# hasindu2008/cornetto

Measured on AMD Instinct MI355X. Metric: Gbases/s scanned (telowin+sdust+boringbits), higher is better.
Workload: dtype u8/u16 integer

## Files before the change

cornetto_amd/csrc/cov.hip:

```cpp
#include <algorithm>
#include <cmath>

#include "common.hpp"
#include "scan.hpp"
#include "tiles.hpp"
#include "ivlmerge.hpp"
#include "internal.hpp"

namespace {

constexpr int CB_THREADS = 256;
#ifndef CN_CB_PARTS
#define CN_CB_PARTS 2
#endif
constexpr int CB_PARTS = CN_CB_PARTS;
constexpr int CB_MAX_INC_LDS = 128;

struct CbArgs {
    const uint16_t *depth, *mq;
    const int64_t *ctg_off;
    const int32_t *ctg_len;
    const int2 *tiles;
    int32_t inc, r;
    uint2 *pre;
    uint2 *head;
    int64_t n_tiles;
    const int4 *tmeta;
    uint2 *tile_tot32;
    ulonglong2 *tile_tot64;
};

typedef unsigned short cb_us2 __attribute__((ext_vector_type(2)));
__device__ __forceinline__ uint32_t add_u16x2(uint32_t acc, uint32_t pair)
{
    const cb_us2 ones = {1, 1};
    return __builtin_amdgcn_udot2(__builtin_bit_cast(cb_us2, pair), ones, acc, false);
}

typedef unsigned int cb_u4 __attribute__((ext_vector_type(4)));

template <bool STAGE, int INC, int NT = 1>
__global__ __launch_bounds__(CB_THREADS) void cov_blocks(CbArgs A)
{
    __builtin_amdgcn_s_setprio(CN_STREAM_PRIO);

    extern __shared__ __attribute__((aligned(16))) uint8_t smem[];
    __shared__ uint32_t wsum[2][CB_THREADS / 64];
    __shared__ unsigned long long wsum64[2][CB_THREADS / 64];

    const int t = threadIdx.x;
    const int inc = INC ? INC : A.inc, r = A.r;
    constexpr int PBc = CB_THREADS / CB_PARTS;
    constexpr int NVIc = INC ? (PBc * INC / 8 + CB_THREADS - 1) / CB_THREADS : 4;
    cb_u4 pre_all[NT][2][CB_PARTS][NVIc];
    if (STAGE && INC) {
#pragma unroll
        for (int ti = 0; ti < NT; ++ti) {
            const int64_t tix = (int64_t)blockIdx.x * NT + ti;
            if (tix >= A.n_tiles) continue;
            int2 tl;
            int ln;
            int64_t of;
            if (A.tmeta) {
                const int4 m0 = A.tmeta[2 * tix], m1 = A.tmeta[2 * tix + 1];
                tl = make_int2(m0.x, m0.y); ln = m0.z; of = (int64_t)(((unsigned long long)(uint32_t)m1.y << 32) | (uint32_t)m1.x);
            } else {
                tl = A.tiles[tix]; ln = A.ctg_len[tl.x]; of = A.ctg_off[tl.x];
            }
            const int64_t e0l = (int64_t)tl.y * inc;
            const int nvec = PBc * inc / 8;
#pragma unroll
            for (int which = 0; which < 2; ++which)
#pragma unroll
                for (int part = 0; part < CB_PARTS; ++part) {
                    const int64_t pe0 = e0l + (int64_t)part * PBc * inc;
                    const int64_t left = ((int64_t)ln - pe0) * 2;
                    const uint32_t nrec = left <= 0 ? 0u : (uint32_t)(left < (int64_t)nvec * 16 ? (left + 15) & ~15LL : (int64_t)nvec * 16);
                    const __amdgpu_buffer_rsrc_t rs = __builtin_amdgcn_make_buffer_rsrc((void *)((which ? A.mq : A.depth) + of + pe0), 0, (int)nrec, 0x00020000);
#pragma unroll
                    for (int k = 0; k < NVIc; ++k) pre_all[ti][which][part][k] = __builtin_amdgcn_raw_buffer_load_b128(rs, (t + k * CB_THREADS) * 16, 0, 0);
                }
        }
    }
#pragma unroll
  for (int ti = 0; ti < NT; ++ti) {
    const int64_t tix = (int64_t)blockIdx.x * NT + ti;
    if (tix >= A.n_tiles) break;
    if (ti) __syncthreads();
    int2 tile;
    int len;
    int64_t off;
    if (A.tmeta) {
        const int4 m0 = A.tmeta[2 * tix], m1 = A.tmeta[2 * tix + 1];
        tile = make_int2(m0.x, m0.y); len = m0.z; off = (int64_t)(((unsigned long long)(uint32_t)m1.y << 32) | (uint32_t)m1.x);
    } else {
        tile = A.tiles[tix]; len = A.ctg_len[tile.x]; off = A.ctg_off[tile.x];
    }
    const int64_t e0 = (int64_t)tile.y * inc;
    const int64_t p0 = e0 + (int64_t)t * inc;

    uint32_t fd = 0, fq = 0, hd = 0, hq = 0;
    unsigned long long xd = 0, xq = 0;
    if (STAGE) {
        uint16_t *sv = reinterpret_cast<uint16_t *>(smem);
        constexpr int PB = CB_THREADS / CB_PARTS;
        const int nvec = PB * inc / 8;
        const int base = (t % PB) * inc;
        const int nval = p0 >= len ? 0 : (int)(len - p0 < inc ? len - p0 : inc);
        const int nh = r < nval ? r : nval;
        constexpr int NVI = NVIc;
        auto &pre = pre_all[ti];
#pragma unroll
        for (int which = 0; which < 2; ++which) {
#pragma unroll
            for (int part = 0; part < CB_PARTS; ++part) {
                const int64_t pe0 = e0 + (int64_t)part * PB * inc;
                const int64_t left = ((int64_t)len - pe0) * 2;
                const uint32_t nrec = left <= 0 ? 0u : (uint32_t)(left < (int64_t)nvec * 16 ? (left + 15) & ~15LL : (int64_t)nvec * 16);
                const __amdgpu_buffer_rsrc_t rs = __builtin_amdgcn_make_buffer_rsrc((void *)((which ? A.mq : A.depth) + off + pe0), 0, (int)nrec, 0x00020000);
                if (which | part) __syncthreads();
                constexpr int NV = 4;
                if (INC) {
#pragma unroll
                    for (int k = 0; k < NVI; ++k) {
                        const int v = t + k * CB_THREADS;
                        if (v < nvec) reinterpret_cast<cb_u4 *>(sv)[v] = pre[which][part][k];
                    }
                } else
                for (int v0 = t; v0 < nvec; v0 += NV * CB_THREADS) {
                    cb_u4 a[NV];
#pragma unroll
                    for (int k = 0; k < NV; ++k) a[k] = __builtin_amdgcn_raw_buffer_load_b128(rs, (v0 + k * CB_THREADS) * 16, 0, 0);
#pragma unroll
                    for (int k = 0; k < NV; ++k) {
                        const int v = v0 + k * CB_THREADS;
                        if (v < nvec) reinterpret_cast<cb_u4 *>(sv)[v] = a[k];
                    }
                }
                __syncthreads();
                if (t / PB == part) {
                    uint32_t f = 0, hh = 0;
                    if (INC && (INC & 1) == 0 && nval == inc) {
                        const uint32_t *wd = reinterpret_cast<const uint32_t *>(sv + base);
#pragma unroll
                        for (int i = 0; i < (INC ? INC : 2) / 2; ++i) f = add_u16x2(f, wd[i]);
                    } else if (nval == inc && (inc & 1) == 0) {
                        const uint32_t *wd = reinterpret_cast<const uint32_t *>(sv + base);
                        for (int i = 0; i < inc / 2; ++i) f = add_u16x2(f, wd[i]);
                    } else {
#pragma clang loop vectorize(disable) unroll(disable)
                        for (int i = 0; i < nval; ++i) f += sv[base + i];
                    }
#pragma clang loop vectorize(disable) unroll(disable)
                    for (int i = 0; i < nh; ++i) hh += sv[base + i];
                    if (which) { fq = f; hq = hh; } else { fd = f; hd = hh; }
                }
            }
        }
        xd = fd;
        xq = fq;
    } else {
        const uint16_t *d = A.depth + off, *q = A.mq + off;
        for (int64_t p = p0; p < p0 + inc && p < len; ++p) {
            const uint32_t a = d[p], b = q[p];
            xd += a;
            xq += b;
            if (p - p0 < r) {
                hd += a;
                hq += b;
            }
        }
        fd = (uint32_t)xd;
        fq = (uint32_t)xq;
    }

    const int lane = t & 63, wv = t >> 6;
    uint32_t sdv, sqv;
    unsigned long long td = 0, tq = 0;
    if (STAGE) {
        sdv = cnwave::wave_incl_dpp(fd);
        sqv = cnwave::wave_incl_dpp(fq);
    } else {
        sdv = cnwave::wave_incl(fd, lane);
        sqv = cnwave::wave_incl(fq, lane);
        td = xd;
        tq = xq;
#pragma unroll
        for (int d = 32; d >= 1; d >>= 1) {
            td += ((unsigned long long)__shfl_xor((unsigned)(td >> 32), d) << 32) | __shfl_xor((unsigned)td, d);
            tq += ((unsigned long long)__shfl_xor((unsigned)(tq >> 32), d) << 32) | __shfl_xor((unsigned)tq, d);
        }
    }
    if (lane == 63) {
        wsum[0][wv] = sdv;
        wsum[1][wv] = sqv;
    }
    if (!STAGE && lane == 0) {
        wsum64[0][wv] = td;
        wsum64[1][wv] = tq;
    }
    __syncthreads();
    uint32_t pd = 0, pq = 0;
#pragma unroll
    for (int i = 0; i < CB_THREADS / 64; ++i)
        if (i < wv) {
            pd += wsum[0][i];
            pq += wsum[1][i];
        }
    A.pre[(size_t)tix * CB_THREADS + t] = make_uint2(sdv + pd, sqv + pq);
    if (A.r) A.head[(size_t)tix * CB_THREADS + t] = make_uint2(hd, hq);
    if (t == CB_THREADS - 1) {
        A.tile_tot32[tix] = make_uint2(sdv + pd, sqv + pq);
        ulonglong2 x;
        if (STAGE) {
            x.x = sdv + pd;
            x.y = sqv + pq;
        } else {
            x.x = wsum64[0][0] + wsum64[0][1] + wsum64[0][2] + wsum64[0][3];
            x.y = wsum64[1][0] + wsum64[1][1] + wsum64[1][2] + wsum64[1][3];
        }
        A.tile_tot64[tix] = x;
    }
  }
}

__global__ __launch_bounds__(256) void cov_total64(const ulonglong2 *tot64, int64_t n, unsigned long long *grand )
{
    __shared__ unsigned long long sa[4], sb[4];
    unsigned long long a = 0, b = 0;
    for (int64_t i = (int64_t)blockIdx.x * 256 + threadIdx.x; i < n; i += (int64_t)gridDim.x * 256) {
        const ulonglong2 v = tot64[i];
        a += v.x;
        b += v.y;
    }
#pragma unroll
    for (int d = 32; d >= 1; d >>= 1) {
        a += ((unsigned long long)__shfl_xor((unsigned)(a >> 32), d) << 32) | __shfl_xor((unsigned)a, d);
        b += ((unsigned long long)__shfl_xor((unsigned)(b >> 32), d) << 32) | __shfl_xor((unsigned)b, d);
    }
    if ((threadIdx.x & 63) == 0) {
        sa[threadIdx.x >> 6] = a;
        sb[threadIdx.x >> 6] = b;
    }
    __syncthreads();
    if (threadIdx.x == 0) {
        atomicAdd(&grand[0], sa[0] + sa[1] + sa[2] + sa[3]);
        atomicAdd(&grand[1], sb[0] + sb[1] + sb[2] + sb[3]);
    }
}

struct CwArgs {
    const uint2 *pre, *head;
    const uint32_t *toff_d, *toff_q;
    const int64_t *blk_off;
    const int32_t *ctg_len;
    const int32_t *n_reg;
    const int2 *tiles;
    int32_t w, inc, q, r;
    uint32_t w_magic, w_shift;
    int32_t mode;
    int32_t lo, hi, edge, min_len;
    double low_mq;
    cornetto_reg_t *regs;
    cornetto_regrec_t *sel;
    cornetto_regpk_t *pk;
    uint2 *tile_res;
};

__device__ __forceinline__ uint2 cw_prefix(const CwArgs &A, int64_t x)
{
    const uint2 b = A.pre[x];
    return make_uint2(b.x + A.toff_d[x >> 8], b.y + A.toff_q[x >> 8]);
}

__global__ __launch_bounds__(256) void cov_windows(CwArgs A)
{
    __builtin_amdgcn_s_setprio(CN_STREAM_PRIO);

    __shared__ uint32_t wcnt[4];
    const int t = threadIdx.x;
    const int2 tile = A.tiles[blockIdx.x];
    const int ctg = tile.x;
    const int len = A.ctg_len[ctg];
    const int j = tile.y + t;
    bool valid = j < A.n_reg[ctg];
    int st = 0, end = 0, depth = 0, mq = 0;
    bool sel = false;
    if (valid) {
        st = j * A.inc;
        end = st + A.w;
        if (end > len) end = len;
        const int64_t a = A.blk_off[ctg] + j;
        uint32_t sd = 0, sq = 0;
        if (A.q > 0) {
            const uint2 hi = cw_prefix(A, a + A.q - 1);
            uint2 lo = make_uint2(0, 0);
            if (a > 0) lo = cw_prefix(A, a - 1);
            sd = hi.x - lo.x;
            sq = hi.y - lo.y;
        }
        if (A.r) {
            const uint2 hb = A.head[a + A.q];
            sd += hb.x;
            sq += hb.y;
        }
        if (end - st == A.w && A.w_magic && (int32_t)(sd | sq) >= 0) {
            depth = (int32_t)(__umulhi(sd, A.w_magic) >> A.w_shift);
            mq = (int32_t)(__umulhi(sq, A.w_magic) >> A.w_shift);
        } else {
            depth = (int32_t)sd / (end - st);
            mq = (int32_t)sq / (end - st);
        }
        if (A.mode == 0) {
            A.regs[j] = cornetto_reg_t{st, end, depth, mq};
        } else {
            bool fun = depth < A.lo || depth > A.hi;
            if (!fun && !(A.low_mq <= 1.0 && depth > 0 && mq >= depth)) fun = ((double)mq / (double)depth) < A.low_mq;
            if (A.mode == 1) sel = len >= A.min_len && fun;
            else sel = len > A.min_len && st > A.edge && end < len - A.edge && !fun;
        }
    }
    if (A.mode == 0) return;
    const unsigned long long bal = __ballot(sel);
    const int lane = t & 63, wv = t >> 6;
    if (lane == 0) wcnt[wv] = (uint32_t)__popcll(bal);
    __syncthreads();
    uint32_t pre = 0, tot = 0;
#pragma unroll
    for (int i = 0; i < 4; ++i) {
        if (i < wv) pre += wcnt[i];
        tot += wcnt[i];
    }
    if (t == 0) A.tile_res[blockIdx.x] = make_uint2(blockIdx.x * 256u, tot);
    if (sel) {
        const size_t idx = (size_t)blockIdx.x * 256u + pre + __popcll(bal & ((1ull << lane) - 1ull));
        if (A.pk) A.pk[idx] = cornetto_regpk_t{st, (uint16_t)depth, (uint16_t)mq};
        else A.sel[idx] = cornetto_regrec_t{ctg, st, end, depth, mq};
    }
}

__global__ void cov_ctg_first(const uint32_t *ooff, const int32_t *first_tile, int32_t n_ctg, uint32_t n_tiles, const unsigned long long *total, uint32_t *out)
{
    const int32_t i = (int32_t)(blockIdx.x * blockDim.x + threadIdx.x);
    if (i >= n_ctg) return;
    const uint32_t t = (uint32_t)first_tile[i];
    out[i] = t < n_tiles ? ooff[t] : (uint32_t)*total;
}

template <int INTS>
__global__ __launch_bounds__(256) void cov_order(const int32_t *raw, const uint2 *tres, const uint32_t *ooff, int64_t n_tiles, int32_t *dst, const unsigned long long *total,
                                                 uint32_t cap)
{
    const int64_t t = (int64_t)blockIdx.x * 4 + (threadIdx.x >> 6);
    if (t >= n_tiles) return;
    if (*total > cap) return;
    const uint2 r = tres[t];
    const int32_t *src = raw + (size_t)r.x * INTS;
    int32_t *d = dst + (size_t)ooff[t] * INTS;
    const uint32_t nint = r.y * (uint32_t)INTS;
    for (uint32_t i = threadIdx.x & 63; i < nint; i += 64) d[i] = src[i];
}

__global__ __launch_bounds__(256) void cov_order_expand(const cornetto_regpk_t *raw, const uint2 *tres, const uint32_t *ooff, int64_t n_tiles, cornetto_regrec_t *dst,
                                                        const unsigned long long *total, uint32_t cap, const int2 *tiles, const int32_t *ctg_len, int32_t w)
{
    const int64_t t = (int64_t)blockIdx.x * 4 + (threadIdx.x >> 6);
    if (t >= n_tiles) return;
    if (*total > cap) return;
    const uint2 r = tres[t];
    const int32_t ctg = tiles[t].x, len = ctg_len[ctg];
    const cornetto_regpk_t *src = raw + r.x;
    cornetto_regrec_t *d = dst + ooff[t];
    for (uint32_t i = threadIdx.x & 63; i < r.y; i += 64) {
        const cornetto_regpk_t p = src[i];
        const int64_t e = (int64_t)p.st + w;
        d[i] = cornetto_regrec_t{ctg, p.st, e > len ? len : (int32_t)e, (int32_t)p.depth, (int32_t)p.mq_depth};
    }
}

int32_t n_reg_host(int32_t length, int32_t w, int32_t inc)
{
    int32_t n = (length - w + inc - 1) / inc + 1;
    return n < 1 ? 1 : n;
}

int32_t regs_assert_host(int32_t length, int32_t w, int32_t inc)
{
    const int64_t st = (int64_t)(n_reg_host(length, w, inc) - 1) * inc;
    int64_t end = st + w;
    if (end > length) end = length;
    if (!(st < end)) return 353;
    return end == length ? 0 : 368;
}

}

extern "C" {

int32_t cornetto_n_reg(int32_t length, int32_t window_size, int32_t window_inc)
{
    if (window_inc <= 0) return 0;
    return n_reg_host(length, window_size, window_inc);
}

int32_t cornetto_regs_assert(int32_t length, int32_t window_size, int32_t window_inc)
{
    if (window_inc <= 0) return 353;
    return regs_assert_host(length, window_size, window_inc);
}

int32_t cornetto_cov_threshold(float factor, int32_t mean)
{
    return (int32_t)round(factor * mean);
}

int cornetto_cov_prepare(cornetto_accel_t *h, cornetto_cov_t *c, int32_t w, int32_t inc, uint64_t sums[3])
{
    if (!h || !c || !sums) return cn_fail(h, CORNETTO_E_ARG, "cov_prepare: bad argument");
    CN_HIP(h, hipSetDevice(h->device));
    cn_timing_begin(h);
    const int rc = cn_cov_prepare_impl(h, c, w, inc, sums);
    if (rc == CORNETTO_OK) cn_timing_end(h);
    return rc;
}

}

struct CwTileFill {
    int2 *out;
    __device__ void operator()(int64_t t, int ci, int64_t j) const { out[t] = make_int2(ci, (int)(j * 256)); }
};
struct CbTileFill {
    int2 *tiles;
    int4 *tmeta;
    const int32_t *len;
    const int64_t *off;
    __device__ void operator()(int64_t t, int ci, int64_t j) const
    {
        const int b = (int)(j * CB_THREADS);
        const unsigned long long o = (unsigned long long)off[ci];
        tiles[t] = make_int2(ci, b);
        tmeta[2 * t] = make_int4(ci, b, len[ci], 0);
        tmeta[2 * t + 1] = make_int4((int)(uint32_t)o, (int)(uint32_t)(o >> 32), 0, 0);
    }
};

int cn_cov_prepare_impl(cornetto_accel_t *h, cornetto_cov_t *c, int32_t w, int32_t inc, uint64_t sums[3])
{
    if (inc < 1) return cn_fail(h, CORNETTO_E_UNSUPPORTED, "cov_prepare: needs window_inc >= 1 (got -i %d: the reference divides by it)", inc);
    for (int32_t i = 0; i < c->n; ++i) {
        const int32_t line = c->len[i] < 1 ? 0 : regs_assert_host(c->len[i], w, inc);
        if (line)
            return cn_fail(h, CORNETTO_E_ASSERT, "src/boringbits_main.c:%d: get_regs: Assertion `%s' failed. (contig %d of length %d, -w %d -i %d)", line,
                           line == 353 ? "st<end" : "end == length", i, c->len[i], w, inc);
    }
    const int32_t q = w / inc, r = w % inc;
    sums[0] = sums[1] = 0;
    sums[2] = (uint64_t)c->total;
    CN_TRACE("cov_prepare: enter");
    if (c->w != w || c->inc != inc || !c->d_blk) {
        struct Invalidate {
            cornetto_cov_t *c;
            bool keep = false;
            ~Invalidate() { if (!keep) c->w = c->inc = -1; }
        } built{c};
        c->w = w;
        c->inc = inc;
        c->cw_mode = -1;
        c->blk_off.assign(c->n + 1, 0);
        c->n_reg.assign(c->n, 0);
        for (int32_t i = 0; i < c->n; ++i) {
            if (c->len[i] < 1) return cn_fail(h, CORNETTO_E_ARG, "cov_prepare: contig %d is empty (a bedgraph cannot produce that)", i);
            c->n_reg[i] = n_reg_host(c->len[i], w, inc);
            c->blk_off[i + 1] = c->blk_off[i] + cn_align_up((int64_t)c->n_reg[i] + q + 1, CB_THREADS);
        }
        c->n_blk = c->blk_off[c->n];
        const int64_t ntl = cntiles::prefix(h, c->cb_pref, c->n, [&](int32_t i) { return (c->blk_off[i + 1] - c->blk_off[i]) / CB_THREADS; });
        if (ntl < 0) return cn_fail(h, CORNETTO_E_NOMEM, "cov_prepare: device allocation failed");
        c->n_cb_tiles = ntl;
        if (c->d_blk) { (void)hipFree(c->d_blk); c->d_blk = nullptr; }
        if (c->d_blk_off) { (void)hipFree(c->d_blk_off); c->d_blk_off = nullptr; }
        if (c->d_cb_tiles) { (void)hipFree(c->d_cb_tiles); c->d_cb_tiles = nullptr; }
        if (c->d_cb_tmeta) { (void)hipFree(c->d_cb_tmeta); c->d_cb_tmeta = nullptr; }
        if (c->d_n_reg) { (void)hipFree(c->d_n_reg); c->d_n_reg = nullptr; }
        const size_t nt = (size_t)ntl;
        if (nt == 0) { built.keep = true; return CORNETTO_OK; }
        if (cn_obj_malloc(h, (void **)&c->d_blk, (size_t)c->n_blk * sizeof(uint4) + 2 * nt * sizeof(uint32_t)) != hipSuccess ||
            cn_obj_malloc(h, (void **)&c->d_blk_off, (size_t)(c->n + 1) * 8) != hipSuccess ||
            cn_obj_malloc(h, (void **)&c->d_cb_tiles, nt * sizeof(int2)) != hipSuccess ||
            cn_obj_malloc(h, (void **)&c->d_cb_tmeta, 2 * nt * sizeof(int4)) != hipSuccess ||
            cn_obj_malloc(h, (void **)&c->d_n_reg, (size_t)c->n * 4) != hipSuccess)
            return cn_fail(h, CORNETTO_E_NOMEM, "cov_prepare: device allocation failed");
        cntiles::fill<<<dim3((unsigned)((nt + 255) / 256)), dim3(256), 0, h->stream>>>(c->cb_pref.dev, c->n, ntl, CbTileFill{c->d_cb_tiles, c->d_cb_tmeta, c->d_len, c->d_off});
        CN_HIP(h, hipGetLastError());
        CN_HIP(h, hipMemcpyAsync(c->d_blk_off, c->blk_off.data(), (size_t)(c->n + 1) * 8, hipMemcpyHostToDevice, h->stream));
        CN_HIP(h, hipMemcpyAsync(c->d_n_reg, c->n_reg.data(), (size_t)c->n * 4, hipMemcpyHostToDevice, h->stream));
        built.keep = true;
    }
    CN_TRACE("cov_prepare: tables");
    const size_t nt = (size_t)c->n_cb_tiles;
    if (nt == 0) return CORNETTO_OK;
    uint2 *d_t32 = (uint2 *)cn_ws(h, WS_CB_T32, nt * sizeof(uint2));
    ulonglong2 *d_t64 = (ulonglong2 *)cn_ws(h, WS_CB_T64, nt * sizeof(ulonglong2));
    unsigned long long *d_grand = (unsigned long long *)cn_ws(h, WS_CB_GRAND, 16);
    unsigned long long *p_grand = (unsigned long long *)cn_pin(h, PIN_SMALL, 64);
    if (!d_t32 || !d_t64 || !d_grand || !p_grand) return cn_fail(h, CORNETTO_E_NOMEM, "cov_prepare: workspace allocation failed");
    uint2 *d_pre = reinterpret_cast<uint2 *>(c->d_blk), *d_head = d_pre + c->n_blk;
    uint32_t *d_toff_d = reinterpret_cast<uint32_t *>(d_head + c->n_blk), *d_toff_q = d_toff_d + nt;
    CN_TRACE("cov_prepare: workspaces");
    CN_HIP(h, hipMemsetAsync(d_grand, 0, 16, h->stream));
    static const int cb_tmeta = CN_DEV_INT("CORNETTO_COV_TMETA", 1);
    CbArgs A{c->d_depth, c->d_mq, c->d_off, c->d_len, c->d_cb_tiles, inc, r, d_pre, d_head, (int64_t)nt, cb_tmeta ? c->d_cb_tmeta : nullptr, d_t32, d_t64};
    if (inc <= CB_MAX_INC_LDS) {
        const size_t lds = (size_t)CB_THREADS / CB_PARTS * inc * sizeof(uint16_t);
        static_assert(CB_THREADS / CB_PARTS * 50 / 8 <= 4 * CB_THREADS, "cov_blocks<true, INC>: at most 4 vectors per thread and part");
        if (A.inc == 50) {
            static const int cb_nt = CN_DEV_INT("CORNETTO_COV_TILES", 1);
            if (cb_nt == 2) {
                CN_HIP(h, hipFuncSetAttribute(reinterpret_cast<const void *>(&cov_blocks<true, 50, 2>), hipFuncAttributeMaxDynamicSharedMemorySize, (int)lds));
                CN_LAUNCH(h, "cov_blocks", cov_blocks<true, 50, 2><<<dim3((unsigned)((nt + 1) / 2)), dim3(CB_THREADS), lds, h->stream>>>(A));
            } else {
                CN_HIP(h, hipFuncSetAttribute(reinterpret_cast<const void *>(&cov_blocks<true, 50>), hipFuncAttributeMaxDynamicSharedMemorySize, (int)lds));
                CN_LAUNCH(h, "cov_blocks", cov_blocks<true, 50><<<dim3((unsigned)nt), dim3(CB_THREADS), lds, h->stream>>>(A));
            }
        } else {
            CN_HIP(h, hipFuncSetAttribute(reinterpret_cast<const void *>(&cov_blocks<true, 0>), hipFuncAttributeMaxDynamicSharedMemorySize, (int)lds));
            CN_LAUNCH(h, "cov_blocks", cov_blocks<true, 0><<<dim3((unsigned)nt), dim3(CB_THREADS), lds, h->stream>>>(A));
        }
    } else {
        CN_LAUNCH(h, "cov_blocks", cov_blocks<false, 0><<<dim3((unsigned)nt), dim3(CB_THREADS), 0, h->stream>>>(A));
    }
    {
        uint32_t *const outs[2] = {d_toff_d, d_toff_q};
        CN_TRY(cnscan::exclusive_u32_multi(h, "cov_tilescan", reinterpret_cast<const uint32_t *>(d_t32), (int64_t)nt, 2, 2, outs, nullptr));
    }
    const unsigned nb64 = (unsigned)std::min<size_t>(1024, (nt + 255) / 256);
    CN_LAUNCH(h, "cov_total64", cov_total64<<<dim3(nb64), dim3(256), 0, h->stream>>>(d_t64, (int64_t)nt, d_grand));
    CN_HIP(h, hipMemcpyAsync(p_grand, d_grand, 16, hipMemcpyDeviceToHost, h->stream));
    CN_TRACE("cov_prepare: queued");
    CN_HIP(h, hipStreamSynchronize(h->stream));
    CN_TRACE("cov_prepare: done");
    sums[0] = p_grand[0] - c->sum_corr[0];
    sums[1] = p_grand[1] - c->sum_corr[1];
    c->sums[0] = sums[0]; c->sums[1] = sums[1]; c->sums[2] = (uint64_t)c->total;
    return CORNETTO_OK;
}

extern "C" {

static int64_t cov_est_key(const cornetto_cov_t *c, int mode, int32_t lo, int32_t hi, float low_mq, int32_t edge, int32_t min_len)
{
    uint32_t qb;
    memcpy(&qb, &low_mq, 4);
    uint64_t k = 1469598103934665603ull;
    for (uint64_t v : {(uint64_t)(uint32_t)mode, (uint64_t)(uint32_t)lo, (uint64_t)(uint32_t)hi, (uint64_t)qb, (uint64_t)(uint32_t)edge, (uint64_t)(uint32_t)min_len,
                       (uint64_t)(uint32_t)c->w, (uint64_t)(uint32_t)c->inc})
        k = (k ^ v) * 1099511628211ull;
    return (int64_t)(k >> 1);
}

static int cov_run_windows(cornetto_accel_t *h, cornetto_cov_t *c, int32_t only_ctg, int mode, int32_t lo, int32_t hi,
                           float low_mq, int32_t edge, int32_t min_len, cornetto_reg_t *regs_host, cornetto_regrec_t **recs,
                           int64_t *n_recs, bool keep_on_device = false, cornetto_regpk_t **pk_out = nullptr, int64_t **ctg_first = nullptr,
                           CnCovSpec *spec = nullptr)
{
    const bool packed = pk_out != nullptr || spec != nullptr;
    CN_TRACE("cov_select: enter");
    const int64_t est_key = cov_est_key(c, mode, lo, hi, low_mq, edge, min_len);
    if (spec) {
        spec->queued = false;
        if (c->cw_est_key != est_key || c->cw_est_cnt < 0) return CORNETTO_OK;
    }
    const size_t rec_bytes = packed ? sizeof(cornetto_regpk_t) : sizeof(cornetto_regrec_t);
    if (!c->d_blk) return cn_fail(h, CORNETTO_E_ARG, "cov: cornetto_cov_prepare() has not been called");
    const int32_t w = c->w, inc = c->inc, q = w / inc, r = w % inc;
    const bool raw_packed = w <= 32768;
    if (packed && !raw_packed) return cn_fail(h, CORNETTO_E_UNSUPPORTED, "cov_select_packed: window size %d > 32768 (a wrapped sum's mean does not fit 16 bits)", w);
    const size_t raw_bytes = raw_packed ? sizeof(cornetto_regpk_t) : sizeof(cornetto_regrec_t);
    if (c->cw_mode != mode || c->cw_min_len != min_len || c->cw_only != only_ctg) {
        const int64_t ntl = cntiles::prefix(h, c->cw_pref, c->n, [&](int32_t i) -> int64_t {
            if (only_ctg >= 0 && i != only_ctg) return 0;
            if (mode == 1 && !(c->len[i] >= min_len)) return 0;
            if (mode == 2 && !(c->len[i] > min_len)) return 0;
            return ((int64_t)c->n_reg[i] + 255) / 256;
        });
        if (ntl < 0) return cn_fail(h, CORNETTO_E_NOMEM, "cov: device allocation failed");
        if (c->d_cw_tiles) { (void)hipFree(c->d_cw_tiles); c->d_cw_tiles = nullptr; }
        if (c->d_cw_first) { (void)hipFree(c->d_cw_first); c->d_cw_first = nullptr; }
        c->n_cw_tiles = ntl;
        if (ntl > 0) {
            c->cw_first.resize((size_t)c->n + 1);
            for (int32_t i = 0; i <= c->n; ++i) c->cw_first[i] = (int32_t)c->cw_pref.host[i];
            if (cn_obj_malloc(h, (void **)&c->d_cw_tiles, (size_t)ntl * sizeof(int2)) != hipSuccess || cn_obj_malloc(h, (void **)&c->d_cw_first, ((size_t)c->n + 1) * 4) != hipSuccess)
                return cn_fail(h, CORNETTO_E_NOMEM, "cov: device allocation failed");
            cntiles::fill<<<dim3((unsigned)((ntl + 255) / 256)), dim3(256), 0, h->stream>>>(c->cw_pref.dev, c->n, ntl, CwTileFill{c->d_cw_tiles});
            CN_HIP(h, hipGetLastError());
            CN_HIP(h, hipMemcpyAsync(c->d_cw_first, c->cw_first.data(), (size_t)c->n * 4, hipMemcpyHostToDevice, h->stream));
        }
        c->cw_mode = mode;
        c->cw_min_len = min_len;
        c->cw_only = only_ctg;
    }
    const size_t nt = (size_t)c->n_cw_tiles;
    if (nt == 0) return CORNETTO_OK;
    const size_t nt_blk = (size_t)c->n_cb_tiles;
    const uint2 *d_pre = reinterpret_cast<const uint2 *>(c->d_blk), *d_head = d_pre + c->n_blk;
    const uint32_t *d_toff_d = reinterpret_cast<const uint32_t *>(d_head + c->n_blk), *d_toff_q = d_toff_d + nt_blk;
    unsigned long long *d_cnt = (unsigned long long *)cn_ws(h, WS_CW_CNT, 16);
    uint2 *d_tres = (uint2 *)cn_ws(h, WS_CW_TRES, nt * 12);
    unsigned long long *p_cnt = spec ? spec->p_cnt : (unsigned long long *)cn_pin(h, PIN_SMALL, 64);
    if (!d_cnt || !d_tres || !p_cnt) return cn_fail(h, CORNETTO_E_NOMEM, "cov: workspace allocation failed");
    uint32_t *d_ooff = reinterpret_cast<uint32_t *>(d_tres + nt);
    CwArgs A{};
    A.pre = d_pre; A.head = d_head; A.toff_d = d_toff_d; A.toff_q = d_toff_q; A.blk_off = c->d_blk_off; A.ctg_len = c->d_len; A.n_reg = c->d_n_reg;
    A.tiles = c->d_cw_tiles; A.w = w; A.inc = inc; A.q = q; A.r = r; A.mode = mode; A.lo = lo; A.hi = hi; A.edge = edge;
    if (w >= 2) {
        int L = 0;
        while ((1ll << L) < (long long)w) ++L;
        A.w_magic = (uint32_t)(((1ull << (31 + L)) / (unsigned long long)w) + 1ull);
        A.w_shift = (uint32_t)(L - 1);
    }
    A.min_len = min_len; A.low_mq = (double)low_mq;
    A.tile_res = d_tres;
    if (mode == 0) {
        const size_t nr = (size_t)c->n_reg[only_ctg];
        cornetto_reg_t *d_regs = (cornetto_reg_t *)cn_ws(h, WS_CW_REGS, nr * sizeof(cornetto_reg_t));
        if (!d_regs) return cn_fail(h, CORNETTO_E_NOMEM, "cov: workspace allocation failed");
        A.regs = d_regs;
        CN_LAUNCH(h, "cov_windows", cov_windows<<<dim3((unsigned)nt), dim3(256), 0, h->stream>>>(A));
        CN_HIP(h, hipMemcpyAsync(regs_host, d_regs, nr * sizeof(cornetto_reg_t), hipMemcpyDeviceToHost, h->stream));
        CN_HIP(h, hipStreamSynchronize(h->stream));
        return CORNETTO_OK;
    }
    const size_t n_raw = nt * 256;
    if (n_raw > 0xffffff00ull) return cn_fail(h, CORNETTO_E_UNSUPPORTED, "cov: %zu window tiles", nt);
    size_t cap = std::max<size_t>(1 << 16, nt * 256 / 8);
    if (h->dev[WS_CW_SEL].bytes > n_raw * raw_bytes) cap = std::max(cap, (h->dev[WS_CW_SEL].bytes - n_raw * raw_bytes) / rec_bytes);
    unsigned long long cnt = 0;
    cornetto_regrec_t *d_raw = nullptr, *d_dst = nullptr;
    uint32_t *p_cf = nullptr, *d_cf = nullptr;
    if (packed) {
        p_cf = (uint32_t *)cn_pin(h, PIN_CW, ((size_t)c->n + 1) * 4);
        d_cf = (uint32_t *)cn_ws(h, WS_CW_CF, ((size_t)c->n + 1) * 4);
        if (!p_cf || !d_cf) return cn_fail(h, CORNETTO_E_NOMEM, "cov_select: allocation failed");
    }
    CN_TRACE("cov_select: tables + small workspaces");
    for (int attempt = 0; attempt < 2; ++attempt) {
        cap = std::min<size_t>(cap, 0x7fffffff);
        d_raw = (cornetto_regrec_t *)cn_ws(h, WS_CW_SEL, n_raw * raw_bytes + cap * rec_bytes);
        if (!d_raw) return cn_fail(h, CORNETTO_E_NOMEM, "cov: workspace allocation of %zu bytes failed", n_raw * raw_bytes + cap * rec_bytes);
        d_dst = reinterpret_cast<cornetto_regrec_t *>(reinterpret_cast<uint8_t *>(d_raw) + n_raw * raw_bytes);
        A.sel = d_raw;
        A.pk = raw_packed ? reinterpret_cast<cornetto_regpk_t *>(d_raw) : nullptr;
        CN_LAUNCH(h, "cov_windows", cov_windows<<<dim3((unsigned)nt), dim3(256), 0, h->stream>>>(A));
        CN_TRY(cnscan::exclusive_u32(h, "cov_order", reinterpret_cast<const uint32_t *>(d_tres) + 1, (int64_t)nt, 2, d_ooff, d_cnt));
        const unsigned nb = (unsigned)((nt + 3) / 4);
        hipEvent_t ea = cn_event(h), eb = cn_event(h);
        (void)hipEventRecord(ea, h->stream);
        if (packed) cov_order<2><<<dim3(nb), dim3(256), 0, h->stream>>>(reinterpret_cast<const int32_t *>(d_raw), d_tres, d_ooff, (int64_t)nt, reinterpret_cast<int32_t *>(d_dst), d_cnt, (uint32_t)cap);
        else if (raw_packed) cov_order_expand<<<dim3(nb), dim3(256), 0, h->stream>>>(reinterpret_cast<const cornetto_regpk_t *>(d_raw), d_tres, d_ooff, (int64_t)nt, d_dst, d_cnt, (uint32_t)cap, c->d_cw_tiles, c->d_len, w);
        else cov_order<5><<<dim3(nb), dim3(256), 0, h->stream>>>(reinterpret_cast<const int32_t *>(d_raw), d_tres, d_ooff, (int64_t)nt, reinterpret_cast<int32_t *>(d_dst), d_cnt, (uint32_t)cap);
        (void)hipEventRecord(eb, h->stream);
        h->recs.push_back(cornetto_accel::Rec{"cov_order", ea, eb});
        if (hipGetLastError() != hipSuccess) return cn_fail(h, CORNETTO_E_HIP, "cov_select: ordering failed");
        if (packed) {
            cov_ctg_first<<<dim3((unsigned)((c->n + 255) / 256)), dim3(256), 0, h->stream>>>(d_ooff, c->d_cw_first, c->n, (uint32_t)nt, d_cnt, d_cf);
            if (hipGetLastError() != hipSuccess || hipMemcpyAsync(p_cf, d_cf, (size_t)c->n * 4, hipMemcpyDeviceToHost, h->stream) != hipSuccess)
                return cn_fail(h, CORNETTO_E_HIP, "cov_select: first records of the contigs failed");
        }
        CN_HIP(h, hipMemcpyAsync(p_cnt, d_cnt, 8, hipMemcpyDeviceToHost, h->stream));
        if (spec) {
            size_t n_copy = std::min<size_t>(cap, (size_t)c->cw_est_cnt + (size_t)c->cw_est_cnt / 16 + 1024);
            if (const int f = CN_DEV_INT("CORNETTO_STEP_EST_FORCE", 0)) n_copy = std::min<size_t>(cap, (size_t)std::max(1, f));
            cornetto_regpk_t *o = (cornetto_regpk_t *)cn_result_alloc(n_copy * rec_bytes);
            if (!o) return cn_fail(h, CORNETTO_E_NOMEM, "cov_select: host allocation failed");
            if (cn_result_d2h(h, o, d_dst, n_copy * rec_bytes) != hipSuccess) {
                cn_result_quiesce(h);
                cornetto_free(o);
                return cn_fail(h, CORNETTO_E_HIP, "cov_select: copy back failed");
            }
            spec->queued = true; spec->o = o; spec->n_copy = n_copy; spec->cap = cap; spec->p_cf = p_cf; spec->key = est_key;
            return CORNETTO_OK;
        }
        CN_HIP(h, hipStreamSynchronize(h->stream));
        cnt = p_cnt[0];
        if (cnt <= cap) break;
        if (attempt == 1 || cnt > 0x7fffffffull) return cn_fail(h, CORNETTO_E_UNSUPPORTED, "cov: %llu selected windows", cnt);
        cap = (size_t)cnt;
    }
    CN_TRACE("cov_select: kernels done, count known");
    cornetto_regrec_t *o = keep_on_device ? d_dst : (cornetto_regrec_t *)cn_result_alloc((cnt ? cnt : 1) * rec_bytes);
    CN_TRACE("cov_select: result block");
    if (!o) return cn_fail(h, CORNETTO_E_NOMEM, "cov_select: host allocation failed");
    if (cnt) {
        if (!keep_on_device && (cn_result_d2h(h, o, d_dst, (size_t)cnt * rec_bytes) != hipSuccess || (!h->lazy && hipStreamSynchronize(h->stream) != hipSuccess))) {
            cn_result_quiesce(h);
            cornetto_free(o);
            return cn_fail(h, CORNETTO_E_HIP, "cov_select: copy back failed");
        }
        if (packed) {
            int64_t *cf = (int64_t *)malloc(((size_t)c->n + 1) * sizeof(int64_t));
            if (!cf) { cn_result_quiesce(h); cornetto_free(o); return cn_fail(h, CORNETTO_E_NOMEM, "cov_select: host allocation failed"); }
            for (int32_t i = 0; i < c->n; ++i) cf[i] = (int64_t)p_cf[i];
            cf[c->n] = (int64_t)cnt;
            *ctg_first = cf;
        }
    } else if (packed) {
        int64_t *cf = (int64_t *)calloc((size_t)c->n + 1, sizeof(int64_t));
        if (!cf) { if (!keep_on_device) cornetto_free(o); return cn_fail(h, CORNETTO_E_NOMEM, "cov_select: host allocation failed"); }
        *ctg_first = cf;
    }
    if (packed) {
        *pk_out = reinterpret_cast<cornetto_regpk_t *>(o);
        c->cw_est_key = est_key;
        c->cw_est_cnt = (int64_t)cnt;
    } else {
        *recs = o;
    }
    *n_recs = (int64_t)cnt;
    return CORNETTO_OK;
}

int cornetto_cov_regs(cornetto_accel_t *h, const cornetto_cov_t *c, int32_t ctg, cornetto_reg_t *regs)
{
    if (!h || !c || !regs || ctg < 0 || ctg >= c->n) return cn_fail(h, CORNETTO_E_ARG, "cov_regs: bad argument");
    CN_HIP(h, hipSetDevice(h->device));
    cn_timing_begin(h);
    int rc = cov_run_windows(h, const_cast<cornetto_cov_t *>(c), ctg, 0, 0, 0, 0.f, 0, 0, regs, nullptr, nullptr);
    cn_timing_end(h);
    return rc;
}

int cornetto_cov_select(cornetto_accel_t *h, const cornetto_cov_t *c, int32_t lo, int32_t hi, float low_mq, int32_t edge_len,
                        int32_t min_ctg_len, int boring, cornetto_regrec_t **recs, int64_t *n_recs)
{
    if (!h || !c || !recs || !n_recs) return cn_fail(h, CORNETTO_E_ARG, "cov_select: bad argument");
    *recs = nullptr;
    *n_recs = 0;
    CN_HIP(h, hipSetDevice(h->device));
    cn_timing_begin(h);
    int rc = cov_run_windows(h, const_cast<cornetto_cov_t *>(c), -1, boring ? 2 : 1, lo, hi, low_mq, edge_len, min_ctg_len, nullptr, recs, n_recs);
    cn_timing_end(h);
    if (rc == CORNETTO_OK && !*recs) {
        *recs = (cornetto_regrec_t *)malloc(sizeof(cornetto_regrec_t));
        if (!*recs) return cn_fail(h, CORNETTO_E_NOMEM, "cov_select: host allocation failed");
    }
    return rc;
}

int cornetto_cov_select_packed(cornetto_accel_t *h, const cornetto_cov_t *c, int32_t lo, int32_t hi, float low_mq, int32_t edge_len,
                               int32_t min_ctg_len, int boring, cornetto_regpk_t **recs, int64_t *n_recs, int64_t **ctg_first)
{
    if (!h || !c || !recs || !n_recs || !ctg_first) return cn_fail(h, CORNETTO_E_ARG, "cov_select_packed: bad argument");
    CN_HIP(h, hipSetDevice(h->device));
    cn_timing_begin(h);
    const int rc = cn_cov_select_packed_impl(h, const_cast<cornetto_cov_t *>(c), lo, hi, low_mq, edge_len, min_ctg_len, boring, recs, n_recs, ctg_first);
    cn_timing_end(h);
    return rc;
}

}

int cn_cov_spec_queue(cornetto_accel_t *h, cornetto_cov_t *c, int32_t lo, int32_t hi, float low_mq, int32_t edge_len, int32_t min_ctg_len, int boring,
                      unsigned long long *p_cnt, CnCovSpec *S)
{
    S->p_cnt = p_cnt;
    return cov_run_windows(h, c, -1, boring ? 2 : 1, lo, hi, low_mq, edge_len, min_ctg_len, nullptr, nullptr, nullptr, false, nullptr, nullptr, S);
}

int cn_cov_spec_finish(cornetto_accel_t *h, cornetto_cov_t *c, CnCovSpec *S, cornetto_regpk_t **recs, int64_t *n_recs, int64_t **ctg_first)
{
    if (!S->queued) return 1;
    S->queued = false;
    const unsigned long long cnt = S->p_cnt[0];
    int64_t *cf = cnt <= S->n_copy ? (int64_t *)malloc(((size_t)c->n + 1) * sizeof(int64_t)) : nullptr;
    if (!cf) {
        cn_result_quiesce(h);
        cornetto_free(S->o);
        S->o = nullptr;
        c->cw_est_key = -1;
        return cnt <= S->n_copy ? cn_fail(h, CORNETTO_E_NOMEM, "cov_select: host allocation failed") : 1;
    }
    for (int32_t i = 0; i < c->n; ++i) cf[i] = (int64_t)S->p_cf[i];
    cf[c->n] = (int64_t)cnt;
    *recs = S->o;
    *n_recs = (int64_t)cnt;
    *ctg_first = cf;
    S->o = nullptr;
    c->cw_est_key = S->key;
    c->cw_est_cnt = (int64_t)cnt;
    return CORNETTO_OK;
}

int cn_cov_select_packed_impl(cornetto_accel_t *h, cornetto_cov_t *c, int32_t lo, int32_t hi, float low_mq, int32_t edge_len, int32_t min_ctg_len, int boring,
                              cornetto_regpk_t **recs, int64_t *n_recs, int64_t **ctg_first)
{
    *recs = nullptr;
    *n_recs = 0;
    *ctg_first = nullptr;
    int rc = cov_run_windows(h, c, -1, boring ? 2 : 1, lo, hi, low_mq, edge_len, min_ctg_len, nullptr, nullptr, n_recs, false, recs, ctg_first);
    if (rc == CORNETTO_OK && !*recs) {
        *recs = (cornetto_regpk_t *)malloc(sizeof(cornetto_regpk_t));
        if (!*ctg_first) *ctg_first = (int64_t *)calloc((size_t)c->n + 1, sizeof(int64_t));
        if (!*recs || !*ctg_first) return cn_fail(h, CORNETTO_E_NOMEM, "cov_select_packed: host allocation failed");
    }
    return rc;
}

extern "C" {

namespace {
__global__ void cov_rec_spans(const cornetto_regrec_t *r, int64_t n, cornetto_ivl_t *out)
{
    const int64_t i = (int64_t)blockIdx.x * blockDim.x + threadIdx.x;
    if (i < n) out[i] = cornetto_ivl_t{r[i].ctg, r[i].st, r[i].end};
}
}

int cornetto_cov_select_merged(cornetto_accel_t *h, const cornetto_cov_t *c, int32_t lo, int32_t hi, float low_mq, int32_t edge_len,
                               int32_t min_ctg_len, int boring, int32_t merge_dist, int32_t min_len, cornetto_ivl_t **ivls, int64_t *n_ivls)
{
    if (!h || !c || !ivls || !n_ivls || merge_dist < 0) return cn_fail(h, CORNETTO_E_ARG, "cov_select_merged: bad argument");
    *ivls = nullptr;
    *n_ivls = 0;
    CN_HIP(h, hipSetDevice(h->device));
    cn_timing_begin(h);
    cornetto_regrec_t *d_recs = nullptr;
    int64_t n = 0;
    CN_TRY(cov_run_windows(h, const_cast<cornetto_cov_t *>(c), -1, boring ? 2 : 1, lo, hi, low_mq, edge_len, min_ctg_len, nullptr, &d_recs, &n, true));
    cornetto_ivl_t *o = nullptr;
    int64_t n_out = 0;
    if (n > 0) {
        uint8_t *ws = (uint8_t *)cn_ws(h, WS_CW_MERGE, cnivl::ws_bytes((size_t)n) + 2 * (size_t)n * sizeof(cornetto_ivl_t));
        unsigned long long *d_cnt = (unsigned long long *)cn_ws(h, WS_CW_CNT, 16);
        unsigned long long *p_cnt = (unsigned long long *)cn_pin(h, PIN_SMALL, 64);
        if (!ws || !d_cnt || !p_cnt) return cn_fail(h, CORNETTO_E_NOMEM, "cov_select_merged: workspace allocation failed");
        cornetto_ivl_t *d_in = (cornetto_ivl_t *)(ws + cnivl::ws_bytes((size_t)n)), *d_out = d_in + n;
        CN_LAUNCH(h, "cov_merge", cov_rec_spans<<<dim3((unsigned)((n + 255) / 256)), dim3(256), 0, h->stream>>>(d_recs, n, d_in));
        CN_TRY(cnivl::merge(h, "cov_merge", d_in, n, merge_dist, ws, d_out, d_cnt + 1));
        CN_HIP(h, hipMemcpyAsync(p_cnt, d_cnt + 1, 8, hipMemcpyDeviceToHost, h->stream));
        CN_HIP(h, hipStreamSynchronize(h->stream));
        const int64_t m = (int64_t)p_cnt[0];
        o = (cornetto_ivl_t *)cn_result_alloc(((size_t)m ? (size_t)m : 1) * sizeof(cornetto_ivl_t));
        if (!o) return cn_fail(h, CORNETTO_E_NOMEM, "cov_select_merged: host allocation failed");
        if (m > 0 && (hipMemcpyAsync(o, d_out, (size_t)m * sizeof(cornetto_ivl_t), hipMemcpyDeviceToHost, h->stream) != hipSuccess ||
                      hipStreamSynchronize(h->stream) != hipSuccess)) {
            cornetto_free(o);
            return cn_fail(h, CORNETTO_E_HIP, "cov_select_merged: copy back failed");
        }
        for (int64_t i = 0; i < m; ++i)
            if (o[i].finish - o[i].start >= min_len) o[n_out++] = o[i];
    }
    cn_timing_end(h);
    if (!o) {
        o = (cornetto_ivl_t *)malloc(sizeof(cornetto_ivl_t));
        if (!o) return cn_fail(h, CORNETTO_E_NOMEM, "cov_select_merged: host allocation failed");
    }
    *ivls = o;
    *n_ivls = n_out;
    return CORNETTO_OK;
}

}
```

Measured before the change: 490.0.

## Add wave-scan coverage block kernel without LDS staging for inc=50

Adds a cov_blocks_scan kernel that loads depth and MAPQ as 128-bit buffer loads straight into registers. It computes per-block prefix sums with a wavefront-wide DPP inclusive scan, using precomputed constant masks that pick where each block of 50 ends inside a vector, and writes results through scattered buffer stores. This removes the LDS staging and transpose of the earlier cov_blocks path, used when inc==50, r==0 and tile metadata is available. It adds a compile-time pattern table, extra lane-mask logic and non-contiguous stores.

```diff
diff --git a/cornetto_amd/csrc/cov.hip b/cornetto_amd/csrc/cov.hip
--- a/cornetto_amd/csrc/cov.hip
+++ b/cornetto_amd/csrc/cov.hip
@@ -222,6 +222,134 @@
         A.tile_tot64[tix] = x;
     }
   }
+}
+
+struct CbsMasks {
+    uint64_t odd[8], hi[8];
+};
+template <int INC>
+struct CbsPattern {
+    static constexpr int NVEC = 64 * INC / 8, NR = (NVEC + 63) / 64;
+    uint32_t off[64][8];
+    uint64_t odd[8], hi[8];
+    constexpr CbsMasks masks() const
+    {
+        CbsMasks m{};
+        for (int k = 0; k < 8; ++k) { m.odd[k] = odd[k]; m.hi[k] = hi[k]; }
+        return m;
+    }
+    constexpr CbsPattern() : off{}, odd{}, hi{}
+    {
+        for (int k = 0; k < 8; ++k)
+            for (int l = 0; l < 64; ++l) {
+                const int v = l + 64 * k, j = (8 * v + 8) / INC, m = j * INC - 8 * v;
+                const bool has = k < NR && v < NVEC && j >= 1 && m >= 2;
+                off[l][k] = has ? (uint32_t)(j - 1) * 8u : 0xFFFFFF00u;
+                if (has && (m == 2 || m == 6)) odd[k] |= 1ull << l;
+                if (has && m >= 6) hi[k] |= 1ull << l;
+            }
+    }
+};
+template <int INC>
+__constant__ const CbsPattern<INC> cbs_pattern{};
+typedef unsigned int cb_u2 __attribute__((ext_vector_type(2)));
+
+__device__ __forceinline__ void cbs_clip(cb_u4 &d, int nv)
+{
+#pragma unroll
+    for (int i = 0; i < 4; ++i) d[i] &= nv >= 2 * i + 2 ? 0xFFFFFFFFu : nv == 2 * i + 1 ? 0x0000FFFFu : 0u;
+}
+
+__device__ __forceinline__ uint32_t cbs_round(const cb_u4 d, uint32_t &carry, uint64_t m_odd, uint64_t m_hi)
+{
+    const uint32_t t1 = add_u16x2(0, d[3]), t2 = add_u16x2(t1, d[2]), t3 = add_u16x2(t2, d[1]), s = add_u16x2(t3, d[0]);
+    const uint32_t incl = cnwave::wave_incl_dpp(s);
+    const bool odd = __builtin_amdgcn_inverse_ballot_w64(m_odd), hi = __builtin_amdgcn_inverse_ballot_w64(m_hi);
+    const uint32_t tail = hi ? (odd ? t1 : 0u) : (odd ? t3 : t2);
+    carry = (uint32_t)__builtin_amdgcn_readlane((int)incl, 63);
+    return incl - tail;
+}
+
+template <int INC>
+__global__ __launch_bounds__(CB_THREADS) void cov_blocks_scan(CbArgs A, CbsMasks M)
+{
+    static_assert(INC >= 8 && INC % 2 == 0 && INC <= 64, "cov_blocks_scan: an even block size, at most one block end per vector, at most 8 rounds");
+    constexpr uint32_t WVALS = 64 * INC;
+    constexpr int NR = CbsPattern<INC>::NR;
+    const int64_t tix = blockIdx.x;
+    const int4 m0 = A.tmeta[2 * tix], m1 = A.tmeta[2 * tix + 1];
+    __shared__ uint32_t wsum[2][CB_THREADS / 64];
+
+    const int lane = threadIdx.x & 63;
+    const uint32_t wv = __builtin_amdgcn_readfirstlane(threadIdx.x >> 6);
+    const int64_t off = (int64_t)(((unsigned long long)(uint32_t)m1.y << 32) | (uint32_t)m1.x);
+    const uint32_t w0 = (uint32_t)m0.y * INC + wv * WVALS, len = (uint32_t)m0.z;
+    const uint32_t rem = w0 >= len ? 0u : len - w0 < WVALS ? len - w0 : WVALS;
+    const uint32_t nrec = (rem * 2 + 15) & ~15u;
+    const int64_t eo = off + w0;
+    const __amdgpu_buffer_rsrc_t rsd = __builtin_amdgcn_make_buffer_rsrc((void *)(A.depth + eo), 0, (int)nrec, 0x00020000);
+    const __amdgpu_buffer_rsrc_t rsq = __builtin_amdgcn_make_buffer_rsrc((void *)(A.mq + eo), 0, (int)nrec, 0x00020000);
+    cb_u4 vd[NR], vq[NR];
+#pragma unroll
+    for (int k = 0; k < NR; ++k) vd[k] = __builtin_amdgcn_raw_buffer_load_b128(rsd, (lane + 64 * k) * 16, 0, 0);
+#pragma unroll
+    for (int k = 0; k < NR; ++k) vq[k] = __builtin_amdgcn_raw_buffer_load_b128(rsq, (lane + 64 * k) * 16, 0, 0);
+    const CbsPattern<INC> &P = cbs_pattern<INC>;
+    const uint4 o0 = *reinterpret_cast<const uint4 *>(&P.off[lane][0]), o1 = *reinterpret_cast<const uint4 *>(&P.off[lane][4]);
+    const uint32_t ooff[8] = {o0.x, o0.y, o0.z, o0.w, o1.x, o1.y, o1.z, o1.w};
+
+    if (rem < WVALS) {
+        const int nv = (int)rem - 8 * lane;
+#pragma unroll
+        for (int k = 0; k < NR; ++k) {
+            cbs_clip(vd[k], nv - 512 * k);
+            cbs_clip(vq[k], nv - 512 * k);
+        }
+    }
+
+    uint32_t cd[NR + 1], cq[NR + 1], od[NR], oq[NR];
+    cd[0] = cq[0] = 0;
+#pragma unroll
+    for (int k = 0; k < NR; ++k) {
+        uint32_t tot;
+        od[k] = cbs_round(vd[k], tot, M.odd[k], M.hi[k]);
+        cd[k + 1] = cd[k] + tot;
+        if (k % 3 == 2 && k + 1 < NR) __builtin_amdgcn_sched_barrier(0);
+    }
+    __builtin_amdgcn_sched_barrier(0);
+#pragma unroll
+    for (int k = 0; k < NR; ++k) {
+        uint32_t tot;
+        oq[k] = cbs_round(vq[k], tot, M.odd[k], M.hi[k]);
+        cq[k + 1] = cq[k] + tot;
+        if (k % 3 == 2 && k + 1 < NR) __builtin_amdgcn_sched_barrier(0);
+    }
+
+    if (lane == 0) {
+        wsum[0][wv] = cd[NR];
+        wsum[1][wv] = cq[NR];
+    }
+    __syncthreads();
+    const bool front = (uint32_t)(lane & 3) < wv;
+    const uint32_t wd = wsum[0][lane & 3], wq = wsum[1][lane & 3];
+    uint32_t fd = front ? wd : 0u, fq = front ? wq : 0u;
+    fd += (uint32_t)__builtin_amdgcn_update_dpp(0, (int)fd, 0xB1, 0xF, 0xF, true);
+    fq += (uint32_t)__builtin_amdgcn_update_dpp(0, (int)fq, 0xB1, 0xF, 0xF, true);
+    fd += (uint32_t)__builtin_amdgcn_update_dpp(0, (int)fd, 0x4E, 0xF, 0xF, true);
+    fq += (uint32_t)__builtin_amdgcn_update_dpp(0, (int)fq, 0x4E, 0xF, 0xF, true);
+    const __amdgpu_buffer_rsrc_t rso = __builtin_amdgcn_make_buffer_rsrc((void *)(A.pre + (size_t)tix * CB_THREADS + wv * 64), 0, 64 * (int)sizeof(uint2), 0x00020000);
+#pragma unroll
+    for (int k = 0; k < NR; ++k) {
+        const cb_u2 o = {od[k] + fd + cd[k], oq[k] + fq + cq[k]};
+        __builtin_amdgcn_raw_buffer_store_b64(o, rso, (int)ooff[k], 0, 0);
+    }
+    if (wv == CB_THREADS / 64 - 1 && lane == 0) {
+        A.tile_tot32[tix] = make_uint2(cd[NR] + fd, cq[NR] + fq);
+        ulonglong2 x;
+        x.x = cd[NR] + fd;
+        x.y = cq[NR] + fq;
+        A.tile_tot64[tix] = x;
+    }
 }
 
 __global__ __launch_bounds__(256) void cov_total64(const ulonglong2 *tot64, int64_t n, unsigned long long *grand )
@@ -514,7 +642,9 @@
     if (inc <= CB_MAX_INC_LDS) {
         const size_t lds = (size_t)CB_THREADS / CB_PARTS * inc * sizeof(uint16_t);
         static_assert(CB_THREADS / CB_PARTS * 50 / 8 <= 4 * CB_THREADS, "cov_blocks<true, INC>: at most 4 vectors per thread and part");
-        if (A.inc == 50) {
+        if (A.inc == 50 && r == 0 && A.tmeta && !CN_DEV_INT("CORNETTO_COV_BLOCKS_STAGE", 0)) {
+            CN_LAUNCH(h, "cov_blocks", cov_blocks_scan<50><<<dim3((unsigned)nt), dim3(CB_THREADS), 0, h->stream>>>(A, CbsPattern<50>{}.masks()));
+        } else if (A.inc == 50) {
             static const int cb_nt = CN_DEV_INT("CORNETTO_COV_TILES", 1);
             if (cb_nt == 2) {
                 CN_HIP(h, hipFuncSetAttribute(reinterpret_cast<const void *>(&cov_blocks<true, 50, 2>), hipFuncAttributeMaxDynamicSharedMemorySize, (int)lds));
```

After: 501.5, median of 6. No clear change (+2.4%).
